# The-Learning-And-Vision-Atelier-LAVA/BUFFER

Measured on AMD Instinct MI355X. Metric: registration pairs/sec, higher is better.
Workload: dtype f32

## Files before the change

buffer_amd/_lib.py:

```python
import ctypes as C
import os

_HERE = os.path.dirname(os.path.abspath(__file__))
LIB_PATH = os.environ.get("BUF_LIB_PATH") or os.path.join(_HERE, "libbuffer_hip.so")

BUF_OK = 0


class BufferHipError(RuntimeError):
    pass


class buf_grid_t(C.Structure):
    _fields_ = [
        ("ws", C.c_void_p), ("ws_bytes", C.c_size_t),
        ("ns", C.c_int), ("nb", C.c_int),
        ("cells_per_elem", C.c_int64),
        ("radius", C.c_float),
        ("supports", C.c_void_p),
        ("desc", C.c_void_p), ("s_off", C.c_void_p), ("table", C.c_void_p),
        ("sorted", C.c_void_p), ("order", C.c_void_p), ("scan_tmp", C.c_void_p),
    ]


# ... 27 lines not shown
    "buf_select_patches_batched": (_i, [_vp, _vp, _i, _vp, _i, _f, _i, _vp, _vp, _sz, _vp]),
    "buf_permute_clouds": (_i, [_vp, _vp, _vp, _i, _vp, _vp]),
    "buf_compact_ws_bytes": (_sz, [_i]),
    "buf_compact_greater": (_i, [_vp, _i, _i, _f, _vp, _vp, _vp, _sz, _vp]),
    "buf_knn_ws_bytes": (_sz, [_i, _i, _i]),
    "buf_knn1_ws_bytes": (_sz, [_i, _i, _i]),
    "buf_knn": (_i, [_vp, _vp, _i, _i, _i, _i, _i, _vp, _vp, _vp, _sz, _vp]),
    "buf_fps_ragged": (_i, [_vp, _vp, _i, _i, _vp, _vp, _sz, _vp]),
    "buf_svd3x3_batched": (_i, [_vp, _i, _vp, _vp, _vp, _vp]),
    "buf_vn_gather_block": (_i, [_vp, _vp, _vp, _vp, _i, _i, _i, _i, _i, _i, _f, _vp, _vp, _vp, _vp, _f, _vp, _vp]),
    "buf_vn_gather_pre_supported": (_i, [_i, _i, _i]),
    "buf_vn_gather_pre_ws_bytes": (_sz, [_i, _i]),
    "buf_vn_gather_block_pre": (_i, [_vp, _vp, _vp, _vp, _i, _i, _i, _i, _i, _f, _vp, _vp, _vp, _vp, _f, _vp, _vp, _sz, _vp]),
    "buf_vn_pointwise": (_i, [_vp, _vp, _i, _i, _i, _vp, _i, _i, _i, _vp, _vp, _vp, _vp, _f, _vp, _vp, _vp]),
    "buf_gather_max": (_i, [_vp, _vp, _i, _i, _i, _i, _vp, _vp]),
    "buf_vn_std": (_i, [_vp, _vp, _i, _i, _vp, _vp]),
    "buf_score_head_ws_bytes": (_sz, [_i, _i]),
    "buf_score_head": (_i, [_vp, _i, _vp, _i, _vp, _vp, _vp, _vp, _f, _vp, _vp, _vp, _vp, _f, _vp, _vp, _vp, _vp, _vp, _i, _vp, _vp, _i, _f,
                            _vp, _vp, _sz, _vp]),
    "buf_patch_voxelize_ws_bytes": (_sz, [_i]),
    "buf_patch_voxelize": (_i, [_vp, _vp, _i, _i, _f, _vp, _i, _i, _vp, _f, _i, _vp, _vp, _vp, _vp, _vp, _vp, _vp,
                                _vp, _vp, _sz, _vp]),
    "buf_cylindrical_net_wg": (_i, [_vp, _i, _vp, _vp, _vp, _vp, _vp, _vp, _vp]),
    "buf_cylindrical_net_wg_supports": (_i, [_vp, _vp]),
    "buf_cylindrical_net_wg_flags": (_i, [_vp, _vp, _vp]),
    "buf_cylindrical_net_split_safe": (_i, [_vp, _i, _vp, _vp, _vp, _vp, _vp, _vp, _vp, _vp, _vp, _vp, _vp, _vp]),
    "buf_cost_volume_net_split_safe": (_i, [_vp, _vp, _i, _vp, _vp, _i, _vp, _vp, _vp, _vp, _vp, _vp, _vp, _vp]),
    "buf_cylindrical_net_split": (_i, [_vp, _i, _vp, _vp, _vp, _vp, _vp, _vp, _vp, _vp]),
    "buf_cylindrical_net_split_head": (_i, [_vp, _i, _vp, _vp, _vp, _vp, _vp, _vp, _vp, _vp, _vp, _vp]),
    "buf_split_gemm_count": (C.c_longlong, [_i, _i, _i, _i]),
    "buf_split_tile_gemm": (_i, [_vp, _i, _i, _i, _i, _vp]),
    "buf_cost_volume_net_split": (_i, [_vp, _vp, _i, _vp, _vp, _vp, _vp, _vp]),
    "buf_cost_volume_net_split_gather": (_i, [_vp, _i, _vp, _vp, _i, _vp, _vp, _vp, _vp, _vp]),
    "buf_split_filter_count": (C.c_longlong, [_i, _i]),
    "buf_split_tile_filters": (_i, [_vp, _i, _i, _vp]),
    "buf_winograd_tile_weights": (_i, [_vp, _i, _i, _vp]),
    "buf_winograd_f24_tile_weights": (_i, [_vp, _i, _i, _vp]),
    "buf_winograd_group": (_i, [_i, _i]),
    "buf_cost_winograd_group": (_i, [_i]),
    "buf_winograd_tile_filters": (_i, [_vp, _i, _i, _i, _i, _vp]),
    "buf_voxel_downsample_ws_bytes": (_sz, [_i, _i64]),
    "buf_voxel_downsample": (_i, [_vp, _vp, _i, _i, C.c_double, _vp, _vp, _vp, _i64, _vp, _sz, _vp]),
    "buf_voxel_downsample_batch_ws_bytes": (_sz, [_i, _i, _i64]),
    "buf_voxel_downsample_batch": (_i, [_vp, _i, _i, _vp, _i, C.c_double, _vp, _vp, _i64, _vp, _sz, _vp]),
    "buf_knn_normals": (_i, [_vp, _i, _vp, _i, _vp, _i, _i, _vp, _i, _vp, _vp, _vp]),
    "buf_icp_ws_bytes": (_sz, [_i, _i, _i, _i]),
    "buf_icp_batched": (_i, [_vp, _vp, _vp, _vp, _vp, _i, _i, _f, _vp, _i, C.c_double, C.c_double, _vp, _vp, _vp, _vp, _vp,
                             _vp, _sz, _vp]),
    "buf_gicp_batched": (_i, [_vp, _vp, _vp, _vp, _vp, _vp, _i, _f, C.c_double, _vp, _i, C.c_double, C.c_double, _vp, _vp, _vp, _vp,
# ... 55 lines not shown
```

buffer_amd/csrc/buffer_hip.hip:

```cpp
#include <stdlib.h>
#include "core.hip"
#include "radius.hip"
#include "icp.hip"
#include "pairstats.hip"
#include "posegraph.hip"
#include "metrics.hip"
#include "subsample.hip"
#include "pointops.hip"
#include "vn.hip"
#include "voxelize.hip"
#include "registration.hip"
#include "convnet.hip"
#include "convnet_h3.hip"
#include "costnet_h3.hip"
#include "preprocess.hip"
#include "convnet_wg.hip"
#include "convnet_w24.hip"
#include "convnet_w24k.hip"
#include "costnet.hip"
#include "split_safe.hip"
#include "fpfh.hip"
#include "fgr.hip"
```

buffer_amd/csrc/convnet_w24.hip:

```cpp
#include "common.h"

#define W24_WSTRIDE 768
#define W24_SET_F22(CIN) (16 * 128 * (CIN))

__device__ __forceinline__ void w24_tile(int li, int& ty, int& tx)
{
    const bool last = li == 15;
    ty = last ? 3 : li / 5;
    tx = last ? 4 : li - 5 * ty;
}

__device__ __forceinline__ unsigned w24_row_addr(unsigned act_addr, int a, int li, int lk)
{
    int ty, tx;
    w24_tile(li, ty, tx);
    const int row = 2 * ty - 1 + a;
    return act_addr + 4u * (unsigned)(lk * WG_CS + ((row >= 0 && row <= 6) ? row * WG_ROW + 4 * tx : WG_ZERO));
}

struct W24AddrPark { float a[4]; };
__device__ __forceinline__ void w24_park_addresses(const float* act, int li, int lk, W24AddrPark& pk)
{
    const unsigned act_addr = (unsigned)(size_t)(__attribute__((address_space(3))) const float*)act;
#pragma unroll
// ... 376 lines not shown
{
    for (int l = 0; l < WG_LAYERS; l++) {
        BUF_REQUIRE(relu[l] >= 0 && relu[l] <= (BUF_CYL_F24K | WG_F24_FLAG | 1), BUF_EINVAL,
                    "buf_cylindrical_net_wg: layer %d has the relu word %d (bit 0: ReLU, bits 1 and 2: the F(2x4) flags, nothing above)", l, relu[l]);
        BUF_REQUIRE(!(relu[l] & BUF_CYL_F24K) || (cout[l] == 64 && cin[l] % 64 == 0), BUF_EINVAL,
                    "buf_cylindrical_net_wg: the K-split F(2x4) flag (bit 2) goes only on layers with 64 output channels and Cin %% 64 == 0 "
                    "(layer %d: %d -> %d, flags %d)", l, cin[l], cout[l], relu[l]);
        BUF_REQUIRE(((relu[l] & WG_F24_FLAG) != 0) == (cout[l] == 128), BUF_EINVAL,
                    "buf_cylindrical_net_wg: the F(2x4) flag goes on every layer with 128 output channels and on no other (layer %d: %d -> %d, flags %d)",
                    l, cin[l], cout[l], relu[l]);
    }
    return BUF_OK;
}

extern "C" int buf_cylindrical_net_wg_flags(const int* cin_host, const int* cout_host, const int* relu_host)
{
    BUF_REQUIRE(cin_host && cout_host && relu_host, BUF_EINVAL, "buf_cylindrical_net_wg_flags: null argument");
    if (int rc = wg_check_widths(cin_host, cout_host)) return rc;
    for (int l = 0; l < WG_LAYERS; l++)
        if (relu_host[l] >= 2) return w24_check_flags(cin_host, cout_host, relu_host);
    return BUF_OK;
}

static int w24k_launch(const float* x, int npatch, CylWgParams P, float* y, void* stream);
static int w24_launch(const float* x, int npatch, CylWgParams P, float* y, void* stream)
{
    if (int rc = w24_check_flags(P.cin, P.cout, P.relu)) return rc;
    bool ksplit = false;
    for (int l = 0; l < WG_LAYERS; l++) {
        if (P.relu[l] & WG_F24_FLAG) P.wt[l] += W24_SET_F22(P.cin[l]);
        ksplit |= (P.relu[l] & BUF_CYL_F24K) != 0;
        P.relu[l] &= ~WG_F24_FLAG;
    }
    if (ksplit) return w24k_launch(x, npatch, P, y, stream);
    size_t lds = sizeof(float) * WG_BUF;
    static LdsGrant grant, grant_rerun;
    if (int rc = P.only_if ? grant_dynamic_lds((const void*)k_cyl_net_w24_rerun, lds, grant_rerun) : grant_dynamic_lds((const void*)k_cyl_net_w24, lds, grant)) return rc;
    double macs = 0;
    for (int l = 0; l < WG_LAYERS; l++) macs += 9.0 * P.cin[l] * P.cout[l];
    TimedSpan span;
    bool timed = !P.only_if && timing_begin((hipStream_t)stream, &span, 2.0 * 140 * macs * npatch, BUF_TIMED_CYL_NET);
    if (P.only_if) k_cyl_net_w24_rerun<<<npatch, WG_THREADS, lds, (hipStream_t)stream>>>(x, P, y);
    else k_cyl_net_w24<<<npatch, WG_THREADS, lds, (hipStream_t)stream>>>(x, P, y);
    if (timed) timing_end((hipStream_t)stream, &span);
    BUF_LAUNCH_CHECK();
    return BUF_OK;
}
```

buffer_amd/csrc/convnet_wg.hip:

```cpp
#include "common.h"
#include <type_traits>

#define WG_CS 160
#define WG_ROW 22
#define WG_ZERO 154
#define WG_MAXC 128
#define WG_LAYERS 8
#define WG_THREADS 256
#define WG_BUF (WG_MAXC * WG_CS)
#define WG_KSTEP (16 * WG_CS)
#define WG_BLOCKS 16

typedef float wgf4 __attribute__((ext_vector_type(4)));
typedef float wgf2 __attribute__((ext_vector_type(2)));
typedef const __attribute__((address_space(3))) wgf2* wg_lds_f2;

struct CylWgParams {
    const float* wt[WG_LAYERS];
    const float* bias[WG_LAYERS];
    int cin[WG_LAYERS], cout[WG_LAYERS], relu[WG_LAYERS];
    const int* only_if;
#ifdef WG_STAMP
    long long* stamps;
#endif
// ... 599 lines not shown
        const int ci = cin[l], co = cout[l];
        BUF_REQUIRE(ci > 0 && ci % 16 == 0 && ci <= WG_MAXC && (co == 32 || co == 64 || co == 128), BUF_EINVAL,
                    "buf_cylindrical_net_wg: layer %d has unsupported widths %d -> %d", l, ci, co);
        BUF_REQUIRE(co != 128 || ci % 32 == 0, BUF_EINVAL,
                    "buf_cylindrical_net_wg: layer %d has unsupported widths %d -> %d (128 output channels need Cin %% 32 == 0)", l, ci, co);
        BUF_REQUIRE(co != 32 || (ci % 32 == 0 && ci <= 64), BUF_EINVAL,
                    "buf_cylindrical_net_wg: layer %d has unsupported widths %d -> %d (32 output channels need Cin = 32 or 64)", l, ci, co);
        BUF_REQUIRE(l == 0 || ci == cout[l - 1], BUF_EINVAL, "buf_cylindrical_net_wg: layer %d width mismatch", l);
        BUF_REQUIRE(l == 0 || cout[l - 1] != 32 || co == 32, BUF_EINVAL,
                    "buf_cylindrical_net_wg: layer %d has unsupported widths %d -> %d (only 32-output layers may follow a 32-output layer)", l, ci, co);
    }
    BUF_REQUIRE(cout[WG_LAYERS - 1] == 32, BUF_EINVAL, "buf_cylindrical_net_wg: the last layer must have 32 channels");
    return BUF_OK;
}

extern "C" int buf_cylindrical_net_wg_supports(const int* cin_host, const int* cout_host)
{
    BUF_REQUIRE(cin_host && cout_host, BUF_EINVAL, "buf_cylindrical_net_wg_supports: null argument");
    return wg_check_widths(cin_host, cout_host);
}

#define WG_F24_FLAG BUF_CYL_F24
static inline bool wg_f24_flagged(int relu) { return relu >= 2; }
static int w24_launch(const float* x, int npatch, CylWgParams P, float* y, void* stream);

static int wg_launch(const float* x, int npatch, const float* const* wt_host, const float* const* bias_host, const int* cin_host,
                     const int* cout_host, const int* relu_host, float* y, const int* only_if, void* stream)
{
    BUF_REQUIRE(npatch >= 0, BUF_EINVAL, "buf_cylindrical_net_wg: npatch=%d", npatch);
    if (npatch == 0) return BUF_OK;
    BUF_REQUIRE(x && y && wt_host && bias_host && cin_host && cout_host && relu_host, BUF_EINVAL, "buf_cylindrical_net_wg: null argument");
    CylWgParams P;
    for (int l = 0; l < WG_LAYERS; l++) {
        P.wt[l] = wt_host[l]; P.bias[l] = bias_host[l];
        P.cin[l] = cin_host[l]; P.cout[l] = cout_host[l]; P.relu[l] = relu_host[l];
        BUF_REQUIRE(P.wt[l] && P.bias[l], BUF_EINVAL, "buf_cylindrical_net_wg: null weights for layer %d", l);
    }
    if (int rc = wg_check_widths(P.cin, P.cout)) return rc;
    P.only_if = only_if;
    for (int l = 0; l < WG_LAYERS; l++)
        if (wg_f24_flagged(relu_host[l])) return w24_launch(x, npatch, P, y, stream);
    size_t lds = sizeof(float) * WG_BUF;
    static LdsGrant grant, grant_rerun;
    if (int rc = only_if ? grant_dynamic_lds((const void*)k_cyl_net_wg_rerun, lds, grant_rerun) : grant_dynamic_lds((const void*)k_cyl_net_wg, lds, grant)) return rc;
    double macs = 0;
    for (int l = 0; l < WG_LAYERS; l++) macs += 9.0 * P.cin[l] * P.cout[l];
    TimedSpan span;
    bool timed = !only_if && timing_begin((hipStream_t)stream, &span, 2.0 * 140 * macs * npatch, BUF_TIMED_CYL_NET);
#ifdef WG_STAMP
    BUF_CHECK_HIP(hipMalloc(&P.stamps, (size_t)npatch * (4 * 20 + 4) * sizeof(long long)));
#endif
    if (only_if) k_cyl_net_wg_rerun<<<npatch, WG_THREADS, lds, (hipStream_t)stream>>>(x, P, y);
    else k_cyl_net_wg<<<npatch, WG_THREADS, lds, (hipStream_t)stream>>>(x, P, y);
    if (timed) timing_end((hipStream_t)stream, &span);
    BUF_LAUNCH_CHECK();
#ifdef WG_STAMP
    {
        BUF_CHECK_HIP(hipStreamSynchronize((hipStream_t)stream));
        long long* h = (long long*)malloc((size_t)npatch * (4 * 20 + 4) * sizeof(long long));
        BUF_CHECK_HIP(hipMemcpy(h, P.stamps, (size_t)npatch * (4 * 20 + 4) * sizeof(long long), hipMemcpyDeviceToHost));
        double comp[WG_LAYERS][4] = {}, wait[WG_LAYERS][4] = {}, tot = 0, pre = 0; long n = 0;
        for (int b = npatch / 2; b < npatch; b++, n++)
            for (int w = 0; w < 4; w++) {
                const long long* q = h + ((size_t)b * 4 + w) * 20;
// ... 1 lines not shown
                if (w == 0) { tot += (double)(q[2 * WG_LAYERS] - q[0]); pre += (double)(q[0] - q[17]); }
            }
        if (n && npatch >= 1024) {
            double dc = 0, dr = 0;
            for (int b = npatch / 2; b < npatch; b++) { const long long* q = h + (size_t)npatch * 80 + (size_t)b * 4; dc += (double)(q[2] - q[0]); dr += (double)(q[3] - q[1]); }
            fprintf(stderr, "  WG_STAMP in-kernel clock: %.0f shader cycles per workgroup over %.0f ticks of the 100 MHz counter -> %.3f GHz\n", dc / n, dr / n, dc / dr * 0.1);
            fprintf(stderr, "WG_STAMP: %ld workgroups, layers total %.0f cycles per patch, input phase %.0f\n", n, tot / n, pre / n);
            for (int l = 0; l < WG_LAYERS; l++) {
                const double mf = 38.0 * (P.cin[l] / 4) * (P.cout[l] / 16) / 4;
                fprintf(stderr, "  layer %d %3d->%3d: MFMAs/wave %5.0f | to barrier %7.0f %7.0f %7.0f %7.0f | wait %6.0f %6.0f %6.0f %6.0f | cycles per MFMA slot %.1f\n",
                        l, P.cin[l], P.cout[l], mf, comp[l][0] / n, comp[l][1] / n, comp[l][2] / n, comp[l][3] / n, wait[l][0] / n, wait[l][1] / n,
                        wait[l][2] / n, wait[l][3] / n, (comp[l][0] + wait[l][0]) / n / (2 * mf));
            }
        }
        free(h); (void)hipFree(P.stamps);
    }
#endif
    return BUF_OK;
}

extern "C" int buf_cylindrical_net_wg(const float* x, int npatch, const float* const* wt_host, const float* const* bias_host,
                                      const int* cin_host, const int* cout_host, const int* relu_host, float* y, void* stream)
{
    return wg_launch(x, npatch, wt_host, bias_host, cin_host, cout_host, relu_host, y, nullptr, stream);
}
```

buffer_amd/csrc/core.hip:

```cpp
#include "common.h"
#include <stdarg.h>

static thread_local char g_err[512] = "";

void buf_set_error(const char* fmt, ...)
{
    va_list ap;
    va_start(ap, fmt);
    vsnprintf(g_err, sizeof(g_err), fmt, ap);
    va_end(ap);
}

extern "C" const char* buf_last_error(void) { return g_err; }
extern "C" int buf_version(void) { return 630; }

#include <mutex>
#include <vector>
struct TimedSpan { hipEvent_t a, b; double bytes; int id; };
static std::mutex g_time_mu;
static std::vector<TimedSpan> g_spans;
static int g_timing_on = 0;

extern "C" void buf_timing_enable(int on) { std::lock_guard<std::mutex> l(g_time_mu); g_timing_on = on; }

static bool timing_begin(hipStream_t s, TimedSpan* sp, double bytes, int id = BUF_TIMED_GRID_QUERY)
{
    if (!g_timing_on) return false;
    sp->id = id;
    if (hipEventCreate(&sp->a) != hipSuccess || hipEventCreate(&sp->b) != hipSuccess) return false;
    sp->bytes = bytes;
    (void)hipEventRecord(sp->a, s);
    return true;
}

static void timing_end(hipStream_t s, TimedSpan* sp)
{
    (void)hipEventRecord(sp->b, s);
// ... 233 lines not shown
```

buffer_amd/csrc/split_safe.hip:

```cpp
#include "common.h"

extern "C" int buf_cylindrical_net_split_safe(const float* x, int npatch, const void* const* wt_split_host, const float* const* wt_wg_host,
                                              const float* const* bias_host, const int* cin_host, const int* cout_host, const int* relu_host,
                                              const float* head_params, float* y_or_equi, float* desc, int* status_dev, int* flags_ws,
                                              void* stream)
{
    BUF_REQUIRE(npatch >= 0, BUF_EINVAL, "buf_cylindrical_net_split_safe: npatch=%d", npatch);
    if (npatch == 0) return BUF_OK;
    BUF_REQUIRE(x && y_or_equi && flags_ws && wt_split_host && wt_wg_host && bias_host && cin_host && cout_host && relu_host, BUF_EINVAL,
                "buf_cylindrical_net_split_safe: null argument");
    BUF_REQUIRE(!head_params || desc, BUF_EINVAL, "buf_cylindrical_net_split_safe: head without desc");
    if (int rc = buf_cylindrical_net_wg_flags(cin_host, cout_host, relu_host)) return rc;
    hipStream_t s = (hipStream_t)stream;
    BUF_CHECK_HIP(hipMemsetAsync(flags_ws, 0, sizeof(int) * (size_t)npatch, s));
    int relu_split[WG_LAYERS];
    for (int l = 0; l < WG_LAYERS; l++) relu_split[l] = wg_f24_flagged(relu_host[l]) ? (relu_host[l] & 1) : relu_host[l];
    int rc = h3_launch(x, npatch, wt_split_host, bias_host, cin_host, cout_host, relu_split, head_params ? nullptr : y_or_equi, head_params,
                       desc, head_params ? y_or_equi : nullptr, status_dev, stream, flags_ws);
    if (rc) return rc;
    rc = wg_launch(x, npatch, wt_wg_host, bias_host, cin_host, cout_host, relu_host, y_or_equi, flags_ws, stream);
    if (rc) return rc;
    if (head_params) {
        k_desc_head_masked<<<npatch, DH_THREADS, 0, s>>>(y_or_equi, head_params, desc, y_or_equi, flags_ws);
        BUF_LAUNCH_CHECK();
    }
    return BUF_OK;
}

extern "C" int buf_cost_volume_net_split_safe(const float* s_eq, const float* t_eq, int ele_n, const long long* s_rows, const long long* t_rows,
                                              int m, const void* const* wt_split_host, const float* const* bias_split_host,
                                              const float* const* wt_f32_host, const float* const* bias_f32_host, float* ind_out,
                                              int* status_dev, int* flags_ws, void* stream)
{
    BUF_REQUIRE(m >= 0, BUF_EINVAL, "buf_cost_volume_net_split_safe: m=%d", m);
    if (m == 0) return BUF_OK;
    BUF_REQUIRE(s_eq && t_eq && wt_split_host && bias_split_host && wt_f32_host && bias_f32_host && ind_out && flags_ws, BUF_EINVAL,
                "buf_cost_volume_net_split_safe: null argument");
    BUF_REQUIRE((s_rows == nullptr) == (t_rows == nullptr), BUF_EINVAL, "buf_cost_volume_net_split_safe: one row list without the other");
    BUF_REQUIRE(!s_rows || ele_n == 7, BUF_EINVAL, "buf_cost_volume_net_split_safe: ele_n=%d (the kernels are built for ele_n = 7)", ele_n);
    hipStream_t s = (hipStream_t)stream;
    BUF_CHECK_HIP(hipMemsetAsync(flags_ws, 0, sizeof(int) * (size_t)m, s));
    int rc = cost_net_h3_launch(s_eq, t_eq, m, wt_split_host, bias_split_host, s_rows, t_rows, ele_n, ind_out, status_dev, stream,
                                "buf_cost_volume_net_split_safe", flags_ws);
    if (rc) return rc;
    return cost_net_launch(s_eq, t_eq, m, wt_f32_host, bias_f32_host, s_rows, t_rows, ele_n, ind_out, stream, "buf_cost_volume_net_split_safe", flags_ws);
}
```

buffer_amd/ops.py:

```python
import ctypes as C
import time
import os
import numpy as np
import torch

from . import _lib
from ._lib import buf_grid_t, check


def _stream():
    return C.c_void_p(torch.cuda.current_stream().cuda_stream)


def _dev(t, dtype, what):
    if not isinstance(t, torch.Tensor) or not t.is_cuda:
        raise _lib.BufferHipError(f"{what}: expected a tensor in device memory (buffer_amd has no CPU path)")
    if t.dtype != dtype:
        t = t.to(dtype)
    return t.contiguous()


def _ptr(t):
    return C.c_void_p(t.data_ptr()) if t is not None else C.c_void_p(0)

# ... 682 lines not shown
    U = np.transpose(U, (2, 0, 5, 3, 6, 4, 1))
    lead = U.shape[:3]
    wide = U[..., [0, 1, 2, 5]].reshape(*lead, 512)
    narrow = U[..., [3, 4]].reshape(*lead, 256)
    return np.ascontiguousarray(np.concatenate([wide, narrow], axis=-1), dtype=np.float32).reshape(-1)


F24_G2 = np.array([[1, 0, 0], [.5, .5, .5], [.5, -.5, .5], [0, 0, 1]], np.float64)
F24_G4 = np.array([[.25, 0, 0], [-1 / 6, -1 / 6, -1 / 6], [-1 / 6, 1 / 6, -1 / 6], [1 / 24, 1 / 12, 1 / 6], [1 / 24, -1 / 12, 1 / 6], [0, 0, 1]],
                  np.float64)


def winograd_f24_filters(w):
    w64 = np.asarray(w, np.float64)
    U = np.zeros((4, 6) + w64.shape[:2], np.float64)
    for a in range(3):
        for b in range(3):
            U += (F24_G2[:, a][:, None, None, None] * w64[None, None, :, :, a, b]) * F24_G4[:, b][None, :, None, None]
    return U


F24_FLAG = 2
F24K_FLAG = 4


def cyl_layer_filters(w, f24k=True):
    wt = winograd_tile_weights(w)
    cout, cin = w.shape[0], w.shape[1]
    if cout == 128:
        flag = F24_FLAG
    elif f24k and cout == 64 and cin % 64 == 0:
        flag = F24K_FLAG
    else:
        return wt, 0
    return np.concatenate([wt, winograd_f24_tile_weights(w)]), flag


class CylindricalNet:

    def __init__(self, layers, device, f24=True, f24k=True):
        self.wt, self.bias, self.cin, self.cout, self.relu = [], [], [], [], []
        self.entry = "buf_cylindrical_net_wg"
        flags = []
        for w, b, relu in layers:
            cout, cin = w.shape[0], w.shape[1]
            wt, flag = cyl_layer_filters(w, f24k) if f24 else (winograd_tile_weights(w), 0)
            flags.append(flag)
            self.wt.append(torch.from_numpy(wt).to(device))
            self.bias.append(torch.from_numpy(np.ascontiguousarray(b, dtype=np.float32)).to(device))
            self.cin.append(cin); self.cout.append(cout); self.relu.append(1 if relu else 0)
        n = len(layers)
        self._wp = (C.c_void_p * n)(*[t.data_ptr() for t in self.wt])
        self._bp = (C.c_void_p * n)(*[t.data_ptr() for t in self.bias])
        self._ci = (C.c_int * n)(*self.cin)
        self._co = (C.c_int * n)(*self.cout)
        self._re = (C.c_int * n)(*[r | f for r, f in zip(self.relu, flags)])

    def __call__(self, x):
        L = _lib.lib()
        x = x.contiguous()
        P = x.shape[0]
        y = torch.empty((P, self.cout[-1], 7, 20), dtype=torch.float32, device=x.device)
        check(L.buf_cylindrical_net_wg(_ptr(x), P, self._wp, self._bp, self._ci, self._co, self._re, _ptr(y), _stream()), self.entry)
        return y


def split_tile_filters(w):
    L = _lib.lib()
    w = np.ascontiguousarray(w, dtype=np.float32)
    cout, cin = w.shape[0], w.shape[1]
    out = np.empty(L.buf_split_filter_count(cout, cin), dtype=np.uint16)
    check(L.buf_split_tile_filters(w.ctypes.data, cout, cin, out.ctypes.data), "buf_split_tile_filters")
    return out


class CylindricalNetSplit:

    def __init__(self, layers, device, f24k=True):
        self.wt, self.bias, self.cin, self.cout, self.relu = [], [], [], [], []
        self.entry = "buf_cylindrical_net_split"
        for w, b, relu in layers:
            cout, cin = w.shape[0], w.shape[1]
            self.wt.append(torch.from_numpy(split_tile_filters(w).view(np.int16)).to(device))
            self.bias.append(torch.from_numpy(np.ascontiguousarray(b, dtype=np.float32)).to(device))
            self.cin.append(cin); self.cout.append(cout); self.relu.append(1 if relu else 0)
        n = len(layers)
        self.status = torch.zeros(1, dtype=torch.int32, device=device)
        self._wp = (C.c_void_p * n)(*[t.data_ptr() for t in self.wt])
        self._bp = (C.c_void_p * n)(*[t.data_ptr() for t in self.bias])
        self._ci = (C.c_int * n)(*self.cin)
        self._co = (C.c_int * n)(*self.cout)
        self._re = (C.c_int * n)(*self.relu)
        self.last_flags = None
        self.safe = n == 8 and _lib.lib().buf_cylindrical_net_wg_supports(self._ci, self._co) == 0 and not os.environ.get('BUF_SPLIT_UNSAFE')
        if self.safe:
            tiled = [cyl_layer_filters(w, f24k) for w, _, _ in layers]
            self.wt_wg = [torch.from_numpy(wt).to(device) for wt, _ in tiled]
            self._wwp = (C.c_void_p * n)(*[t.data_ptr() for t in self.wt_wg])
            self._re_safe = (C.c_int * n)(*[r | f for r, (_, f) in zip(self.relu, tiled)])

    def _safe_call(self, x, head):
        L = _lib.lib()
        x = x.contiguous()
        P = x.shape[0]
        out = torch.empty((P, self.cout[-1], 7, 20), dtype=torch.float32, device=x.device)
        desc = torch.empty((P, 32), dtype=torch.float32, device=x.device) if head is not None else None
        self.last_flags = torch.empty((max(P, 1),), dtype=torch.int32, device=x.device)
        check(L.buf_cylindrical_net_split_safe(_ptr(x), P, self._wp, self._wwp, self._bp, self._ci, self._co, self._re_safe,
                                               _ptr(head.params) if head is not None else None, _ptr(out), _ptr(desc), _ptr(self.status),
                                               _ptr(self.last_flags), _stream()), "buf_cylindrical_net_split_safe")
        return (desc, out) if head is not None else out

    def __call__(self, x):
        if self.safe:
            return self._safe_call(x, None)
        L = _lib.lib()
        x = x.contiguous()
        P = x.shape[0]
        y = torch.empty((P, self.cout[-1], 7, 20), dtype=torch.float32, device=x.device)
        check(L.buf_cylindrical_net_split(_ptr(x), P, self._wp, self._bp, self._ci, self._co, self._re, _ptr(y), _ptr(self.status), _stream()),
              self.entry)
        return y

    def with_head(self, x, head):
        if self.safe:
            return self._safe_call(x, head)
        L = _lib.lib()
        x = x.contiguous()
        P = x.shape[0]
        desc = torch.empty((P, 32), dtype=torch.float32, device=x.device)
        equi = torch.empty((P, 32, 7, 20), dtype=torch.float32, device=x.device)
        check(L.buf_cylindrical_net_split_head(_ptr(x), P, self._wp, self._bp, self._ci, self._co, self._re, _ptr(head.params),
                                               _ptr(desc), _ptr(equi), _ptr(self.status), _stream()), "buf_cylindrical_net_split_head")
# ... 183 lines not shown
```

include/buffer_hip.h:

```cpp
#ifndef BUFFER_HIP_H
#define BUFFER_HIP_H
#include <stddef.h>
#include <stdint.h>
#ifdef __cplusplus
extern "C" {
#endif

#define BUF_OK            0
#define BUF_EINVAL       -1
#define BUF_EHIP         -2
#define BUF_EWORKSPACE   -3
#define BUF_ECAPACITY    -4
#define BUF_ENODEVICE    -5

const char* buf_last_error(void);
int         buf_version(void);
int         buf_device_count(void);
#define BUF_TIMED_GRID_QUERY 0
#define BUF_TIMED_CYL_NET    1
#define BUF_TIMED_COST_NET   2
#define BUF_TIMED_SELECT_PATCHES 3
#define BUF_TIMED_PATCH_VOXELIZE 4
#define BUF_TIMED_FPS            5
#define BUF_TIMED_NN1            6
// ... 95 lines not shown
int     buf_score_head(const float* x, int n, const int* lens_host, int nseg,
                       const float* vn1_wf, const float* vn1_wd, const float* vn1_bsc, const float* vn1_bsh, float vn1_slope,
                       const float* vn2_wf, const float* vn2_wd, const float* vn2_bsc, const float* vn2_bsh, float vn2_slope,
                       const float* lin, const float* w0, const float* b0, const float* w1, const float* b1, int c1,
                       const float* w2, const float* b2, int final_activation, float eps, float* out,
                       void* ws, size_t ws_bytes, void* stream);

size_t  buf_patch_voxelize_ws_bytes(int ncentres);
int     buf_patch_voxelize(const float* patches, const float* axis, int npatch, int npts, float des_r,
                           const float* centres, int ncentres, int azi_n, const float* azi_cs, float voxel_r,
                           int nsample, const float* mlp_w_host, const float* mlp_b_host, const float* bn_scale_host,
                           const float* bn_shift_host, float* out_x, float* out_R, float* out_rand, float* out_patches,
                           void* ws, size_t ws_bytes, void* stream);

int     buf_winograd_group(int cin, int cout);
int     buf_winograd_tile_weights(const float* w_host, int cout, int cin, float* out_host);
int     buf_winograd_tile_filters(const float* w_host, int cout, int cin, int ng, int nblk, float* out_host);
#define BUF_CYL_F24 2
#define BUF_CYL_F24K 4
int     buf_cylindrical_net_wg_flags(const int* cin_host, const int* cout_host, const int* relu_host);
int     buf_winograd_f24_tile_weights(const float* w_host, int cout, int cin, float* out_host);
int     buf_cylindrical_net_wg(const float* x, int npatch, const float* const* wt_host, const float* const* bias_host,
                               const int* cin_host, const int* cout_host, const int* relu_host, float* y, void* stream);
int     buf_cylindrical_net_wg_supports(const int* cin_host, const int* cout_host);

long long buf_split_filter_count(int cout, int cin);
int     buf_split_tile_filters(const float* w_host, int cout, int cin, unsigned short* out_host);
int     buf_cylindrical_net_split(const float* x, int npatch, const void* const* wt_host, const float* const* bias_host,
                                  const int* cin_host, const int* cout_host, const int* relu_host, float* y, int* status_dev, void* stream);
int     buf_cylindrical_net_split_head(const float* x, int npatch, const void* const* wt_host, const float* const* bias_host,
                                       const int* cin_host, const int* cout_host, const int* relu_host, const float* head_params,
                                       float* desc, float* equi, int* status_dev, void* stream);

int     buf_cylindrical_net_split_safe(const float* x, int npatch, const void* const* wt_split_host, const float* const* wt_wg_host,
                                       const float* const* bias_host, const int* cin_host, const int* cout_host, const int* relu_host,
                                       const float* head_params, float* y_or_equi, float* desc, int* status_dev, int* flags_ws, void* stream);

int     buf_descriptor_head(const float* y, int npatch, const float* params, float* desc, float* equi, void* stream);

int     buf_cost_winograd_group(int layer);
int     buf_cost_volume_net(const float* s_eq, const float* t_eq, int m, const float* const* wt_host,
                            const float* const* bias_host, float* ind_out, void* stream);
int     buf_cost_volume_net_gather(const float* equi, int ele_n, const long long* s_rows, const long long* t_rows, int m,
                                   const float* const* wt_host, const float* const* bias_host, float* ind_out, void* stream);

long long buf_split_gemm_count(int cout, int cin, int ntaps, int nt);
int     buf_split_tile_gemm(const float* w_host, int cout, int cin, int ntaps, int nt, unsigned short* out_host);
int     buf_cost_volume_net_split(const float* s_eq, const float* t_eq, int m, const void* const* wt_host,
                                  const float* const* bias_host, float* ind_out, int* status_dev, void* stream);
int     buf_cost_volume_net_split_gather(const float* equi, int ele_n, const long long* s_rows, const long long* t_rows, int m,
                                         const void* const* wt_host, const float* const* bias_host, float* ind_out,
                                         int* status_dev, void* stream);
int     buf_cost_volume_net_split_safe(const float* s_eq, const float* t_eq, int ele_n, const long long* s_rows, const long long* t_rows,
                                       int m, const void* const* wt_split_host, const float* const* bias_split_host,
                                       const float* const* wt_f32_host, const float* const* bias_f32_host, float* ind_out,
                                       int* status_dev, int* flags_ws, void* stream);

int     buf_hypotheses_score(const float* ind, const float* ss_kpts, const float* tt_kpts, const float* ss_R,
                             const float* tt_R, int m, int azi_n, float inlier_th, float* R_out, float* t_out,
// ... 95 lines not shown
```

Baseline: 166.7.

## Add pass-split Winograd F(2,4) layer form for cout-64 cylindrical conv layers

Adds a new kernel variant (w24p) for the cout=64 K-split Winograd layers. Each wave computes a different input-transform pass over all output tiles and the partial results are exchanged through LDS, instead of splitting the reduction over input channels. A separate direct path handles the border row. The new form becomes the library and Python default, and form-selecting entry points are added. The aim is better MFMA utilisation and less reduction overhead, at the cost of an LDS exchange and extra synchronisation.

```diff
diff --git a/buffer_amd/_lib.py b/buffer_amd/_lib.py
--- a/buffer_amd/_lib.py
+++ b/buffer_amd/_lib.py
@@ -73,9 +73,11 @@
     "buf_patch_voxelize": (_i, [_vp, _vp, _i, _i, _f, _vp, _i, _i, _vp, _f, _i, _vp, _vp, _vp, _vp, _vp, _vp, _vp,
                                 _vp, _vp, _sz, _vp]),
     "buf_cylindrical_net_wg": (_i, [_vp, _i, _vp, _vp, _vp, _vp, _vp, _vp, _vp]),
+    "buf_cylindrical_net_wg_form": (_i, [_vp, _i, _vp, _vp, _vp, _vp, _vp, _i, _vp, _vp]),
     "buf_cylindrical_net_wg_supports": (_i, [_vp, _vp]),
     "buf_cylindrical_net_wg_flags": (_i, [_vp, _vp, _vp]),
     "buf_cylindrical_net_split_safe": (_i, [_vp, _i, _vp, _vp, _vp, _vp, _vp, _vp, _vp, _vp, _vp, _vp, _vp, _vp]),
+    "buf_cylindrical_net_split_safe_form": (_i, [_vp, _i, _vp, _vp, _vp, _vp, _vp, _vp, _i, _vp, _vp, _vp, _vp, _vp, _vp]),
     "buf_cost_volume_net_split_safe": (_i, [_vp, _vp, _i, _vp, _vp, _i, _vp, _vp, _vp, _vp, _vp, _vp, _vp, _vp]),
     "buf_cylindrical_net_split": (_i, [_vp, _i, _vp, _vp, _vp, _vp, _vp, _vp, _vp, _vp]),
     "buf_cylindrical_net_split_head": (_i, [_vp, _i, _vp, _vp, _vp, _vp, _vp, _vp, _vp, _vp, _vp, _vp]),
diff --git a/buffer_amd/csrc/buffer_hip.hip b/buffer_amd/csrc/buffer_hip.hip
--- a/buffer_amd/csrc/buffer_hip.hip
+++ b/buffer_amd/csrc/buffer_hip.hip
@@ -17,6 +17,7 @@
 #include "convnet_wg.hip"
 #include "convnet_w24.hip"
 #include "convnet_w24k.hip"
+#include "convnet_w24p.hip"
 #include "costnet.hip"
 #include "split_safe.hip"
 #include "fpfh.hip"
diff --git a/buffer_amd/csrc/convnet_w24.hip b/buffer_amd/csrc/convnet_w24.hip
--- a/buffer_amd/csrc/convnet_w24.hip
+++ b/buffer_amd/csrc/convnet_w24.hip
@@ -422,8 +422,10 @@
     return BUF_OK;
 }
 
+#define BUF_CYL_FORM_LIBRARY BUF_CYL_FORM_PASS_SPLIT
 static int w24k_launch(const float* x, int npatch, CylWgParams P, float* y, void* stream);
-static int w24_launch(const float* x, int npatch, CylWgParams P, float* y, void* stream)
+static int w24p_launch(const float* x, int npatch, CylWgParams P, float* y, void* stream);
+static int w24_launch(const float* x, int npatch, CylWgParams P, float* y, void* stream, int form)
 {
     if (int rc = w24_check_flags(P.cin, P.cout, P.relu)) return rc;
     bool ksplit = false;
@@ -432,7 +434,8 @@
         ksplit |= (P.relu[l] & BUF_CYL_F24K) != 0;
         P.relu[l] &= ~WG_F24_FLAG;
     }
-    if (ksplit) return w24k_launch(x, npatch, P, y, stream);
+    if (form == BUF_CYL_FORM_DEFAULT) form = BUF_CYL_FORM_LIBRARY;
+    if (ksplit) return form == BUF_CYL_FORM_PASS_SPLIT ? w24p_launch(x, npatch, P, y, stream) : w24k_launch(x, npatch, P, y, stream);
     size_t lds = sizeof(float) * WG_BUF;
     static LdsGrant grant, grant_rerun;
     if (int rc = P.only_if ? grant_dynamic_lds((const void*)k_cyl_net_w24_rerun, lds, grant_rerun) : grant_dynamic_lds((const void*)k_cyl_net_w24, lds, grant)) return rc;
diff --git a/buffer_amd/csrc/convnet_w24p.hip b/buffer_amd/csrc/convnet_w24p.hip
--- /dev/null
+++ b/buffer_amd/csrc/convnet_w24p.hip
@@ -0,0 +1,311 @@
+#include "common.h"
+
+#define W24P_XCH_C 64
+#define W24P_XCH_WIDE 36
+#define W24P_XCH_OWN 12
+
+#define W24P_MFMA(PRE, ACC, A, B) asm volatile(PRE "v_mfma_f32_16x16x4_f32 %0, %1, %2, %0" : "+a"(ACC) : "v"(A), "v"(B));
+
+__device__ __forceinline__ void w24p_pass(unsigned P0, unsigned P1, float sgn, __amdgpu_buffer_rsrc_t rs, unsigned wp0, unsigned wp1, unsigned wp_next,
+                                          unsigned lofs4, unsigned lofs2, int niter, wgf4 (&W4)[4][2], wgf2 (&W2)[4][2], wgf4 (&acc)[4][6])
+{
+    wgf2 D[6];
+    float V[2][6];
+    W24_LOAD(D, P0, P1, 0)
+#define W24P_XFORM(BUF)                                                                                   \
+    {                                                                                                     \
+        float r_[6];                                                                                      \
+        _Pragma("unroll") for (int b = 0; b < 6; b++)                                                     \
+            r_[b] = __builtin_fmaf(sgn, D[3 + (b >> 1)][b & 1], D[b >> 1][b & 1]);                       \
+        const float c_ = wg_sub(r_[4], r_[2]), e_ = wg_sub(r_[3], r_[1]);                                 \
+        const float a_ = __builtin_fmaf(-4.f, r_[2], r_[4]), b_ = __builtin_fmaf(-4.f, r_[1], r_[3]);     \
+        V[BUF][0] = __builtin_fmaf(4.f, r_[0], __builtin_fmaf(-4.f, r_[2], c_));                          \
+        V[BUF][1] = wg_add(a_, b_); V[BUF][2] = wg_sub(a_, b_);                                           \
+        V[BUF][3] = __builtin_fmaf(2.f, e_, c_); V[BUF][4] = __builtin_fmaf(-2.f, e_, c_);                \
+        V[BUF][5] = __builtin_fmaf(-4.f, e_, wg_sub(r_[5], r_[3]));                                       \
+    }
+    W24P_XFORM(0)
+    int it = 0;
+#pragma unroll 1
+    do {
+        const bool more = it + 1 < niter;
+        const unsigned wcur0 = wp0 + 4 * it * W24_WSTRIDE, wcur1 = wp1 + 4 * it * W24_WSTRIDE;
+        const unsigned wn0 = more ? wcur0 + 4 * W24_WSTRIDE : wp_next;
+        const unsigned wn1 = more ? wcur1 + 4 * W24_WSTRIDE : wp_next;
+        const unsigned adv = more ? 4u * WG_KSTEP : 0u;
+        __builtin_amdgcn_sched_barrier(0);
+#pragma unroll
+        for (int s = 0; s < 4; s++) {
+            if (s < 3) W24_LOAD(D, P0, P1, (s + 1) * WG_KSTEP)
+            else {
+                P0 += adv; P1 += adv;
+                W24_LOAD(D, P0, P1, 0)
+            }
+            __builtin_amdgcn_sched_barrier(0);
+#pragma unroll
+            for (int n = 0; n < 4; n++)
+#pragma unroll
+                for (int j = 0; j < 6; j++) {
+                    if (n == 0 && j == 0) W24P_MFMA("s_nop 1\n\t", acc[n][j], W24_U(n, s & 1, j), V[s & 1][j])
+                    else W24P_MFMA("", acc[n][j], W24_U(n, s & 1, j), V[s & 1][j])
+                }
+            __builtin_amdgcn_sched_barrier(0);
+            W24P_XFORM((s + 1) & 1)
+#pragma unroll
+            for (int n = 0; n < 4; n++) {
+                const unsigned o = n < 2 ? (s < 2 ? wcur0 + (s + 2) * W24_WSTRIDE : wn0 + (s - 2) * W24_WSTRIDE)
+                                         : (s < 2 ? wcur1 + (s + 2) * W24_WSTRIDE : wn1 + (s - 2) * W24_WSTRIDE);
+                W4[n][s & 1] = wg_ldw(rs, o + (n & 1) * 256, lofs4);
+                W2[n][s & 1] = w24_ldw2(rs, o + 512 + (n & 1) * 128, lofs2);
+            }
+            __builtin_amdgcn_sched_barrier(0);
+        }
+    } while (++it < niter);
+#undef W24P_XFORM
+    asm volatile("s_nop 15"
+                 : "+a"(acc[0][0]), "+a"(acc[0][1]), "+a"(acc[0][2]), "+a"(acc[0][3]), "+a"(acc[0][4]), "+a"(acc[0][5]), "+a"(acc[1][0]), "+a"(acc[1][1]), "+a"(acc[1][2]), "+a"(acc[1][3]), "+a"(acc[1][4]), "+a"(acc[1][5]), "+a"(acc[2][0]), "+a"(acc[2][1]), "+a"(acc[2][2]), "+a"(acc[2][3]), "+a"(acc[2][4]), "+a"(acc[2][5]), "+a"(acc[3][0]), "+a"(acc[3][1]), "+a"(acc[3][2]), "+a"(acc[3][3]), "+a"(acc[3][4]), "+a"(acc[3][5]));
+}
+
+__device__ __forceinline__ void w24p_round_direct(unsigned row5, __amdgpu_buffer_rsrc_t rs, unsigned wp, unsigned lofs, int niter, unsigned pstride,
+                                                  const float* __restrict__ bias_lane, const wgf4 (&W0)[2], wgf4& Y)
+{
+    constexpr int wstride = W24_WSTRIDE;
+    wgf4 Wr[3][2];
+#pragma unroll
+    for (int k = 0; k < 2; k++) {
+        Wr[0][k] = W0[k];
+        Wr[1][k] = wg_ldw(rs, wp + pstride + k * wstride, lofs);
+        Wr[2][k] = wg_ldw(rs, wp + 2 * pstride + k * wstride, lofs);
+    }
+    float X[2][6];
+    unsigned pa = row5;
+    WG_LOADD(X[0], pa, 0)
+    WG_LOADD(X[1], pa, WG_KSTEP)
+    wgf4 acc[3];
+    float zero = 0.f;
+    asm volatile("" : "+v"(zero));
+    acc[0] = (wgf4){ zero, zero, zero, zero };
+    acc[1] = (wgf4){ zero, zero, zero, zero };
+    acc[2] = *reinterpret_cast<const wgf4*>(bias_lane);
+    float G[6];
+#define W24P_TAPS(SLOT)                                                                                   \
+    {                                                                                                     \
+        const wgf4 u0_ = Wr[0][SLOT], u1_ = Wr[1][SLOT], u2_ = Wr[2][SLOT];                               \
+        const float d1_ = wg_sub(u1_[1], u2_[1]), d2_ = wg_sub(u1_[2], u2_[2]);                           \
+        G[0] = u0_[0]; G[1] = wg_sub(u0_[1], u0_[2]); G[2] = u0_[3];                                      \
+        G[3] = wg_sub(u1_[0], u2_[0]); G[4] = wg_sub(d1_, d2_); G[5] = wg_sub(u1_[3], u2_[3]);            \
+    }
+#define W24P_RELOAD(SLOT, OFS)                                                                            \
+    _Pragma("unroll") for (int blk = 0; blk < 3; blk++) Wr[blk][SLOT] = wg_ldw(rs, (OFS) + blk * pstride, lofs);
+    W24P_TAPS(0)
+    W24P_RELOAD(0, wp + 2 * wstride)
+#pragma unroll 1
+    for (int it = 0; it < niter; it++) {
+        const bool more = it + 1 < niter;
+        const unsigned wcur = wp + 4 * it * wstride;
+        const unsigned wn = more ? wcur + 4 * wstride : wp;
+        const unsigned adv = more ? 4u * WG_KSTEP : 0u;
+        __builtin_amdgcn_sched_barrier(0);
+#pragma unroll
+        for (int s = 0; s < 4; s++) {
+#pragma unroll
+            for (int a = 0; a < 2; a++)
+#pragma unroll
+                for (int b = 0; b < 3; b++)
+                    acc[b] = __builtin_amdgcn_mfma_f32_16x16x4f32(G[a * 3 + b], X[s & 1][a * 3 + b], acc[b], 0, 0, 0);
+            __builtin_amdgcn_sched_barrier(0);
+            if (s < 2) WG_LOADD(X[s & 1], pa, (s + 2) * WG_KSTEP)
+            else {
+                if (s == 2) pa += adv;
+                WG_LOADD(X[s & 1], pa, (s - 2) * WG_KSTEP)
+            }
+            __builtin_amdgcn_sched_barrier(0);
+            W24P_TAPS((s + 1) & 1)
+            if (s == 0) W24P_RELOAD(1, wcur + 3 * wstride)
+            else W24P_RELOAD((s + 1) & 1, wn + (s - 1) * wstride)
+            __builtin_amdgcn_sched_barrier(0);
+        }
+    }
+#undef W24P_TAPS
+#undef W24P_RELOAD
+#pragma unroll
+    for (int r = 0; r < 4; r++) Y[r] = __builtin_fmaf(4.f, acc[0][r], __builtin_fmaf(-3.f, acc[1][r], acc[2][r]));
+}
+
+template <int W>
+__device__ __forceinline__ void w24p_give(const wgf4 (&f)[4][4], float* __restrict__ act, int lane)
+{
+    float* wide = act + (W24P_XCH_C + 16 * W + (lane >> 2)) * WG_CS + (lane & 3) * W24P_XCH_WIDE;
+#pragma unroll
+    for (int q = 0; q < 4; q++) {
+        if (q == W) continue;
+        const int slot = q - (q > W), rank = W - (W > q);
+#pragma unroll
+        for (int v = 0; v < 3; v++) *reinterpret_cast<wgf4*>(wide + 12 * slot + 4 * v) = f[q][v];
+        *reinterpret_cast<wgf4*>(act + (16 * q + (lane >> 2)) * WG_CS + (lane & 3) * W24P_XCH_OWN + 4 * rank) = f[q][3];
+    }
+}
+
+template <int Q>
+__device__ __forceinline__ void w24p_take(const wgf4 (&f)[4][4], const float* __restrict__ act, int lane, wgf4 (&Yk)[2][4])
+{
+    const float* own = act + (16 * Q + (lane >> 2)) * WG_CS + (lane & 3) * W24P_XCH_OWN;
+#pragma unroll
+    for (int h = 0; h < 2; h++) {
+        wgf4 F[4][2];
+#pragma unroll
+        for (int i = 0; i < 4; i++)
+#pragma unroll
+            for (int v = 2 * h; v < 2 * h + 2; v++) {
+                const int slot = Q - (Q > i), rank = i - (i > Q);
+                const float* wide = act + (W24P_XCH_C + 16 * i + (lane >> 2)) * WG_CS + (lane & 3) * W24P_XCH_WIDE;
+                if (i == Q) F[i][v & 1] = f[Q][v];
+                else if (v < 3) F[i][v & 1] = *reinterpret_cast<const wgf4*>(wide + 12 * slot + 4 * v);
+                else F[i][v & 1] = *reinterpret_cast<const wgf4*>(own + 4 * rank);
+            }
+#pragma unroll
+        for (int v = 2 * h; v < 2 * h + 2; v++) {
+            Yk[0][v] = (F[0][v & 1] + F[1][v & 1]) + F[2][v & 1];
+            Yk[1][v] = (F[1][v & 1] - F[2][v & 1]) - F[3][v & 1];
+        }
+        __builtin_amdgcn_sched_barrier(0);
+    }
+}
+
+__device__ __forceinline__ void w24p_layer_psplit(float* __restrict__ act, const float* __restrict__ wt, const float* __restrict__ bias, int cin, int relu,
+                                                  int w, const WgAddrPark& pk, const W24AddrPark& pk24)
+{
+    act[(threadIdx.x >> 1) * WG_CS + WG_ZERO + 4 + (threadIdx.x & 1)] = 0.f;
+    __syncthreads();
+    int lane = threadIdx.x & (WAVE - 1);
+    asm volatile("" : "+v"(lane));
+    const int lk = lane >> 4;
+    const int k4 = cin >> 2;
+    const __amdgpu_buffer_rsrc_t rs = wg_weights(wt);
+    const unsigned pstride = (unsigned)(k4 * W24_WSTRIDE);
+    const unsigned wp0 = (unsigned)w * pstride, wp1 = wp0 + 4 * pstride;
+    const unsigned wpd = (unsigned)(w >> 1) * 4 * pstride + (unsigned)(w & 1) * 256;
+    const unsigned lofs4 = lane * 16, lofs2 = lane * 8;
+    const wgf4 W0[2] = { wg_ldw(rs, wpd, lofs4), wg_ldw(rs, wpd + W24_WSTRIDE, lofs4) };
+    wgf4 Yb;
+    w24p_round_direct(wg_parked(pk, 2, 0), rs, wpd, lofs4, k4 >> 2, pstride, bias + w * 16 + lk * 4, W0, Yb);
+    unsigned RA[4];
+#pragma unroll
+    for (int a = 0; a < 4; a++) asm volatile("v_accvgpr_read_b32 %0, %1" : "=v"(RA[a]) : "a"(pk24.a[a]));
+    const unsigned P0 = w == 0 ? RA[0] : (w == 2 ? RA[2] : RA[1]);
+    const unsigned P1 = w == 3 ? RA[3] : (w == 2 ? RA[1] : RA[2]);
+    const float sgn = w == 1 ? 1.f : -1.f;
+    wgf4 f[4][4];
+    {
+        wgf4 acc[4][6];
+        float zero = 0.f;
+        asm volatile("" : "+v"(zero));
+#pragma unroll
+        for (int n = 0; n < 4; n++)
+#pragma unroll
+            for (int j = 0; j < 6; j++) acc[n][j] = (wgf4){ zero, zero, zero, zero };
+        if (w == 1) {
+#pragma unroll
+            for (int n = 0; n < 4; n++) acc[n][1] = *reinterpret_cast<const wgf4*>(bias + n * 16 + lk * 4);
+        }
+#pragma unroll
+        for (int n = 0; n < 4; n++)
+#pragma unroll
+            for (int j = 0; j < 6; j++) asm volatile("" : "+a"(acc[n][j]));
+        __builtin_amdgcn_sched_barrier(0);
+        wgf4 W4[4][2];
+        wgf2 W2[4][2];
+#pragma unroll
+        for (int n = 0; n < 4; n++)
+#pragma unroll
+            for (int k = 0; k < 2; k++) {
+                const unsigned o = (n < 2 ? wp0 : wp1) + k * W24_WSTRIDE;
+                W4[n][k] = wg_ldw(rs, o + (n & 1) * 256, lofs4);
+                W2[n][k] = w24_ldw2(rs, o + 512 + (n & 1) * 128, lofs2);
+            }
+        w24p_pass(P0, P1, sgn, rs, wp0, wp1, wp0, lofs4, lofs2, k4 >> 2, W4, W2, acc);
+#pragma unroll
+        for (int n = 0; n < 4; n++)
+#pragma unroll
+            for (int r = 0; r < 4; r++) {
+                const float p = acc[n][1][r] + acc[n][2][r], q = acc[n][1][r] - acc[n][2][r];
+                const float t = acc[n][3][r] + acc[n][4][r], d = acc[n][3][r] - acc[n][4][r];
+                f[n][0][r] = acc[n][0][r] + p + t;
+                f[n][1][r] = __builtin_fmaf(2.f, d, q);
+                f[n][2][r] = __builtin_fmaf(4.f, t, p);
+                f[n][3][r] = __builtin_fmaf(8.f, d, q) + acc[n][5][r];
+            }
+    }
+    __syncthreads();
+    int lane_s = threadIdx.x & (WAVE - 1);
+    asm volatile("" : "+v"(lane_s));
+    if (w == 0) w24p_give<0>(f, act, lane_s);
+    else if (w == 1) w24p_give<1>(f, act, lane_s);
+    else if (w == 2) w24p_give<2>(f, act, lane_s);
+    else w24p_give<3>(f, act, lane_s);
+    __syncthreads();
+    wgf4 Yk[2][4];
+    if (w == 0) w24p_take<0>(f, act, lane_s, Yk);
+    else if (w == 1) w24p_take<1>(f, act, lane_s, Yk);
+    else if (w == 2) w24p_take<2>(f, act, lane_s, Yk);
+    else w24p_take<3>(f, act, lane_s, Yk);
+    w24_store_tile(Yk, w, relu, act, lane_s & 15, lane_s >> 4);
+    wg_store_row6<false>(Yb, w, relu, act, nullptr, lane_s & 15, lane_s >> 4);
+}
+
+__device__ __forceinline__ void cyl_net_w24p_body(const float* __restrict__ x, const CylWgParams& P, float* __restrict__ y, float* __restrict__ lds)
+{
+    float* act = lds;
+    const int patch = blockIdx.x;
+    const int w = __builtin_amdgcn_readfirstlane(threadIdx.x / WAVE);
+    wg_load_input(x, P, act, patch);
+    WgAddrPark pk;
+    W24AddrPark pk24;
+    {
+        int lane0 = threadIdx.x & (WAVE - 1);
+        asm volatile("" : "+v"(lane0));
+        wg_park_addresses(act, lane0 & 15, lane0 >> 4, pk);
+        w24_park_addresses(act, lane0 & 15, lane0 >> 4, pk24);
+    }
+#pragma unroll 1
+    for (int l = 0; l < WG_LAYERS; l++) {
+        const int cin = P.cin[l], cout = P.cout[l], relu = P.relu[l] & 1;
+        if (cout == 128) w24_layer_pair(act, P.wt[l], P.bias[l], cin, relu, w, pk, pk24);
+        else if (cout == 64 && (P.relu[l] & W24K_FLAG)) w24p_layer_psplit(act, P.wt[l], P.bias[l], cin, relu, w, pk, pk24);
+        else if (cout == 64) wg_layer_msplit(act, P.wt[l], P.bias[l], cin, cout, relu, w, pk);
+        else if (l < WG_LAYERS - 1) wg_layer_mksplit<false>(act, nullptr, P.wt[l], P.bias[l], cin, cout, relu, w, pk);
+        else wg_layer_mksplit<true>(act, y + (size_t)patch * cout * 140, P.wt[l], P.bias[l], cin, cout, relu, w, pk);
+        __syncthreads();
+    }
+}
+
+__global__ void __launch_bounds__(WG_THREADS, 2) k_cyl_net_w24p(const float* __restrict__ x, CylWgParams P, float* __restrict__ y)
+{
+    extern __shared__ float lds[];
+    cyl_net_w24p_body(x, P, y, lds);
+}
+
+__global__ void __launch_bounds__(WG_THREADS, 2) k_cyl_net_w24p_rerun(const float* __restrict__ x, CylWgParams P, float* __restrict__ y)
+{
+    extern __shared__ float lds[];
+    if (P.only_if[blockIdx.x] == 0) return;
+    cyl_net_w24p_body(x, P, y, lds);
+}
+
+static int w24p_launch(const float* x, int npatch, CylWgParams P, float* y, void* stream)
+{
+    for (int l = 0; l < WG_LAYERS; l++)
+        if (P.relu[l] & W24K_FLAG) P.wt[l] += WG_BLOCKS * P.cout[l] * P.cin[l];
+    size_t lds = sizeof(float) * WG_BUF;
+    static LdsGrant grant, grant_rerun;
+    if (int rc = P.only_if ? grant_dynamic_lds((const void*)k_cyl_net_w24p_rerun, lds, grant_rerun) : grant_dynamic_lds((const void*)k_cyl_net_w24p, lds, grant)) return rc;
+    double macs = 0;
+    for (int l = 0; l < WG_LAYERS; l++) macs += 9.0 * P.cin[l] * P.cout[l];
+    TimedSpan span;
+    bool timed = !P.only_if && timing_begin((hipStream_t)stream, &span, 2.0 * 140 * macs * npatch, BUF_TIMED_CYL_NET);
+    if (P.only_if) k_cyl_net_w24p_rerun<<<npatch, WG_THREADS, lds, (hipStream_t)stream>>>(x, P, y);
+    else k_cyl_net_w24p<<<npatch, WG_THREADS, lds, (hipStream_t)stream>>>(x, P, y);
+    if (timed) timing_end((hipStream_t)stream, &span);
+    BUF_LAUNCH_CHECK();
+    return BUF_OK;
+}
diff --git a/buffer_amd/csrc/convnet_wg.hip b/buffer_amd/csrc/convnet_wg.hip
--- a/buffer_amd/csrc/convnet_wg.hip
+++ b/buffer_amd/csrc/convnet_wg.hip
@@ -645,12 +645,14 @@
 
 #define WG_F24_FLAG BUF_CYL_F24
 static inline bool wg_f24_flagged(int relu) { return relu >= 2; }
-static int w24_launch(const float* x, int npatch, CylWgParams P, float* y, void* stream);
+static int w24_launch(const float* x, int npatch, CylWgParams P, float* y, void* stream, int form);
 
 static int wg_launch(const float* x, int npatch, const float* const* wt_host, const float* const* bias_host, const int* cin_host,
-                     const int* cout_host, const int* relu_host, float* y, const int* only_if, void* stream)
+                     const int* cout_host, const int* relu_host, float* y, const int* only_if, void* stream, int form)
 {
     BUF_REQUIRE(npatch >= 0, BUF_EINVAL, "buf_cylindrical_net_wg: npatch=%d", npatch);
+    BUF_REQUIRE(form >= BUF_CYL_FORM_DEFAULT && form <= BUF_CYL_FORM_PASS_SPLIT, BUF_EINVAL,
+                "buf_cylindrical_net_wg: form=%d (-1: the library's default, 0: K split, 1: pass split)", form);
     if (npatch == 0) return BUF_OK;
     BUF_REQUIRE(x && y && wt_host && bias_host && cin_host && cout_host && relu_host, BUF_EINVAL, "buf_cylindrical_net_wg: null argument");
     CylWgParams P;
@@ -662,7 +664,7 @@
     if (int rc = wg_check_widths(P.cin, P.cout)) return rc;
     P.only_if = only_if;
     for (int l = 0; l < WG_LAYERS; l++)
-        if (wg_f24_flagged(relu_host[l])) return w24_launch(x, npatch, P, y, stream);
+        if (wg_f24_flagged(relu_host[l])) return w24_launch(x, npatch, P, y, stream, form);
     size_t lds = sizeof(float) * WG_BUF;
     static LdsGrant grant, grant_rerun;
     if (int rc = only_if ? grant_dynamic_lds((const void*)k_cyl_net_wg_rerun, lds, grant_rerun) : grant_dynamic_lds((const void*)k_cyl_net_wg, lds, grant)) return rc;
@@ -710,5 +712,11 @@
 extern "C" int buf_cylindrical_net_wg(const float* x, int npatch, const float* const* wt_host, const float* const* bias_host,
                                       const int* cin_host, const int* cout_host, const int* relu_host, float* y, void* stream)
 {
-    return wg_launch(x, npatch, wt_host, bias_host, cin_host, cout_host, relu_host, y, nullptr, stream);
-}
+    return wg_launch(x, npatch, wt_host, bias_host, cin_host, cout_host, relu_host, y, nullptr, stream, BUF_CYL_FORM_DEFAULT);
+}
+
+extern "C" int buf_cylindrical_net_wg_form(const float* x, int npatch, const float* const* wt_host, const float* const* bias_host,
+                                           const int* cin_host, const int* cout_host, const int* relu_host, int form, float* y, void* stream)
+{
+    return wg_launch(x, npatch, wt_host, bias_host, cin_host, cout_host, relu_host, y, nullptr, stream, form);
+}
diff --git a/buffer_amd/csrc/core.hip b/buffer_amd/csrc/core.hip
--- a/buffer_amd/csrc/core.hip
+++ b/buffer_amd/csrc/core.hip
@@ -12,7 +12,7 @@
 }
 
 extern "C" const char* buf_last_error(void) { return g_err; }
-extern "C" int buf_version(void) { return 630; }
+extern "C" int buf_version(void) { return 640; }
 
 #include <mutex>
 #include <vector>
diff --git a/buffer_amd/csrc/split_safe.hip b/buffer_amd/csrc/split_safe.hip
--- a/buffer_amd/csrc/split_safe.hip
+++ b/buffer_amd/csrc/split_safe.hip
@@ -1,15 +1,17 @@
 #include "common.h"
 
-extern "C" int buf_cylindrical_net_split_safe(const float* x, int npatch, const void* const* wt_split_host, const float* const* wt_wg_host,
-                                              const float* const* bias_host, const int* cin_host, const int* cout_host, const int* relu_host,
-                                              const float* head_params, float* y_or_equi, float* desc, int* status_dev, int* flags_ws,
-                                              void* stream)
+extern "C" int buf_cylindrical_net_split_safe_form(const float* x, int npatch, const void* const* wt_split_host, const float* const* wt_wg_host,
+                                                   const float* const* bias_host, const int* cin_host, const int* cout_host, const int* relu_host,
+                                                   int form, const float* head_params, float* y_or_equi, float* desc, int* status_dev,
+                                                   int* flags_ws, void* stream)
 {
     BUF_REQUIRE(npatch >= 0, BUF_EINVAL, "buf_cylindrical_net_split_safe: npatch=%d", npatch);
     if (npatch == 0) return BUF_OK;
     BUF_REQUIRE(x && y_or_equi && flags_ws && wt_split_host && wt_wg_host && bias_host && cin_host && cout_host && relu_host, BUF_EINVAL,
                 "buf_cylindrical_net_split_safe: null argument");
     BUF_REQUIRE(!head_params || desc, BUF_EINVAL, "buf_cylindrical_net_split_safe: head without desc");
+    BUF_REQUIRE(form >= BUF_CYL_FORM_DEFAULT && form <= BUF_CYL_FORM_PASS_SPLIT, BUF_EINVAL,
+                "buf_cylindrical_net_split_safe: form=%d (-1: the library's default, 0: K split, 1: pass split)", form);
     if (int rc = buf_cylindrical_net_wg_flags(cin_host, cout_host, relu_host)) return rc;
     hipStream_t s = (hipStream_t)stream;
     BUF_CHECK_HIP(hipMemsetAsync(flags_ws, 0, sizeof(int) * (size_t)npatch, s));
@@ -18,13 +20,22 @@
     int rc = h3_launch(x, npatch, wt_split_host, bias_host, cin_host, cout_host, relu_split, head_params ? nullptr : y_or_equi, head_params,
                        desc, head_params ? y_or_equi : nullptr, status_dev, stream, flags_ws);
     if (rc) return rc;
-    rc = wg_launch(x, npatch, wt_wg_host, bias_host, cin_host, cout_host, relu_host, y_or_equi, flags_ws, stream);
+    rc = wg_launch(x, npatch, wt_wg_host, bias_host, cin_host, cout_host, relu_host, y_or_equi, flags_ws, stream, form);
     if (rc) return rc;
     if (head_params) {
         k_desc_head_masked<<<npatch, DH_THREADS, 0, s>>>(y_or_equi, head_params, desc, y_or_equi, flags_ws);
         BUF_LAUNCH_CHECK();
     }
     return BUF_OK;
+}
+
+extern "C" int buf_cylindrical_net_split_safe(const float* x, int npatch, const void* const* wt_split_host, const float* const* wt_wg_host,
+                                              const float* const* bias_host, const int* cin_host, const int* cout_host, const int* relu_host,
+                                              const float* head_params, float* y_or_equi, float* desc, int* status_dev, int* flags_ws,
+                                              void* stream)
+{
+    return buf_cylindrical_net_split_safe_form(x, npatch, wt_split_host, wt_wg_host, bias_host, cin_host, cout_host, relu_host, BUF_CYL_FORM_DEFAULT,
+                                               head_params, y_or_equi, desc, status_dev, flags_ws, stream);
 }
 
 extern "C" int buf_cost_volume_net_split_safe(const float* s_eq, const float* t_eq, int ele_n, const long long* s_rows, const long long* t_rows,
diff --git a/buffer_amd/ops.py b/buffer_amd/ops.py
--- a/buffer_amd/ops.py
+++ b/buffer_amd/ops.py
@@ -728,6 +728,7 @@
 
 F24_FLAG = 2
 F24K_FLAG = 4
+F24P_DEFAULT = True
 
 
 def cyl_layer_filters(w, f24k=True):
@@ -744,9 +745,10 @@
 
 class CylindricalNet:
 
-    def __init__(self, layers, device, f24=True, f24k=True):
+    def __init__(self, layers, device, f24=True, f24k=True, f24p=F24P_DEFAULT):
         self.wt, self.bias, self.cin, self.cout, self.relu = [], [], [], [], []
         self.entry = "buf_cylindrical_net_wg"
+        self.form = 1 if f24p else 0
         flags = []
         for w, b, relu in layers:
             cout, cin = w.shape[0], w.shape[1]
@@ -767,7 +769,7 @@
         x = x.contiguous()
         P = x.shape[0]
         y = torch.empty((P, self.cout[-1], 7, 20), dtype=torch.float32, device=x.device)
-        check(L.buf_cylindrical_net_wg(_ptr(x), P, self._wp, self._bp, self._ci, self._co, self._re, _ptr(y), _stream()), self.entry)
+        check(L.buf_cylindrical_net_wg_form(_ptr(x), P, self._wp, self._bp, self._ci, self._co, self._re, self.form, _ptr(y), _stream()), self.entry)
         return y
 
 
@@ -782,9 +784,10 @@
 
 class CylindricalNetSplit:
 
-    def __init__(self, layers, device, f24k=True):
+    def __init__(self, layers, device, f24k=True, f24p=F24P_DEFAULT):
         self.wt, self.bias, self.cin, self.cout, self.relu = [], [], [], [], []
         self.entry = "buf_cylindrical_net_split"
+        self.form = 1 if f24p else 0
         for w, b, relu in layers:
             cout, cin = w.shape[0], w.shape[1]
             self.wt.append(torch.from_numpy(split_tile_filters(w).view(np.int16)).to(device))
@@ -812,9 +815,9 @@
         out = torch.empty((P, self.cout[-1], 7, 20), dtype=torch.float32, device=x.device)
         desc = torch.empty((P, 32), dtype=torch.float32, device=x.device) if head is not None else None
         self.last_flags = torch.empty((max(P, 1),), dtype=torch.int32, device=x.device)
-        check(L.buf_cylindrical_net_split_safe(_ptr(x), P, self._wp, self._wwp, self._bp, self._ci, self._co, self._re_safe,
-                                               _ptr(head.params) if head is not None else None, _ptr(out), _ptr(desc), _ptr(self.status),
-                                               _ptr(self.last_flags), _stream()), "buf_cylindrical_net_split_safe")
+        check(L.buf_cylindrical_net_split_safe_form(_ptr(x), P, self._wp, self._wwp, self._bp, self._ci, self._co, self._re_safe, self.form,
+                                                    _ptr(head.params) if head is not None else None, _ptr(out), _ptr(desc), _ptr(self.status),
+                                                    _ptr(self.last_flags), _stream()), "buf_cylindrical_net_split_safe_form")
         return (desc, out) if head is not None else out
 
     def __call__(self, x):
diff --git a/include/buffer_hip.h b/include/buffer_hip.h
--- a/include/buffer_hip.h
+++ b/include/buffer_hip.h
@@ -141,6 +141,11 @@
 int     buf_winograd_f24_tile_weights(const float* w_host, int cout, int cin, float* out_host);
 int     buf_cylindrical_net_wg(const float* x, int npatch, const float* const* wt_host, const float* const* bias_host,
                                const int* cin_host, const int* cout_host, const int* relu_host, float* y, void* stream);
+#define BUF_CYL_FORM_DEFAULT (-1)
+#define BUF_CYL_FORM_K_SPLIT 0
+#define BUF_CYL_FORM_PASS_SPLIT 1
+int     buf_cylindrical_net_wg_form(const float* x, int npatch, const float* const* wt_host, const float* const* bias_host,
+                                    const int* cin_host, const int* cout_host, const int* relu_host, int form, float* y, void* stream);
 int     buf_cylindrical_net_wg_supports(const int* cin_host, const int* cout_host);
 
 long long buf_split_filter_count(int cout, int cin);
@@ -154,6 +159,11 @@
 int     buf_cylindrical_net_split_safe(const float* x, int npatch, const void* const* wt_split_host, const float* const* wt_wg_host,
                                        const float* const* bias_host, const int* cin_host, const int* cout_host, const int* relu_host,
                                        const float* head_params, float* y_or_equi, float* desc, int* status_dev, int* flags_ws, void* stream);
+
+int     buf_cylindrical_net_split_safe_form(const float* x, int npatch, const void* const* wt_split_host, const float* const* wt_wg_host,
+                                            const float* const* bias_host, const int* cin_host, const int* cout_host, const int* relu_host,
+                                            int form, const float* head_params, float* y_or_equi, float* desc, int* status_dev, int* flags_ws,
+                                            void* stream);
 
 int     buf_descriptor_head(const float* y, int npatch, const float* params, float* desc, float* equi, void* stream);
 
```

After: 170.0 (median of 6 runs). 1.02x the previous value.
